# 0xMiden/miden-vm

Hardware: AMD Instinct MI355X
Metric: trace rows/sec proved (2^20-row trace, 96-bit sec) (higher is better)
Workload: dtype u64 (Goldilocks field, p = 2^64 - 2^32 + 1); 1 GPU; full proof of miden:20:51:8 (DummyMidenAir 2^20 x 51 + 8 EF aux), 96-bit production PCS params (blowup 8, FRI arity 4, 27 queries, PoW 4/12/16), Poseidon2 LMCS; trace resident in HBM, transcript on host; log_trace_rows=20, main_width=51, aux_width_ef=8, log_blowup=3, proof_bytes=137697, parallelism=1 GPU

## Files before the change

miden-vm_amd/csrc/p2_fast_constants.inc:

```
static const unsigned long long P2F_ARK_INT_SCALED[22] = {
  0x4adf842aa75d4316ULL, 0xc7ddc3945255a751ULL, 0x3a16dbc6b75abaa6ULL, 0x4160d6694e06fff1ULL,
  0xe022996682de326cULL, 0xc8e9d874293bba12ULL, 0xa2e2b15ade3b7d8fULL, 0x9b6dac180ec943cfULL,
  0xe8bb7136f94d695dULL, 0xf12458f8ebe4789bULL, 0x1dc193fff01be2b6ULL, 0xb68e807d90fed489ULL,
  0x1e4085d70c946015ULL, 0x66a5e58521b4c3c6ULL, 0x53b280ba8b2f8249ULL, 0xe4d602af8c2cf37eULL,
  0x813ee2a294c44327ULL, 0x813b943e27068773ULL, 0x9abe7bd4fb69436eULL, 0x12f583e142599766ULL,
  0x3798883e37881f6bULL, 0xed264b0c16fc039fULL,
};
static const unsigned long long P2F_INT_K[22] = {
  0x0000000000000001ULL, 0xffffbfff00004001ULL, 0xefffffff00000001ULL, 0xfffffbff00000001ULL,
  0xfffffffeff000001ULL, 0xfffffffeffffffc1ULL, 0x000ffffffff00000ULL, 0x00000003fffffffcULL,
  0x0001000000000000ULL, 0x0000000040000000ULL, 0x0000000000001000ULL, 0xfbffffff04000001ULL,
  0xfffffeff00000101ULL, 0xffbfffff00000001ULL, 0xffffffef00000001ULL, 0xfffffffefffc0001ULL,
  0xffffffff00000000ULL, 0x00003fffffffc000ULL, 0x1000000000000000ULL, 0x0000040000000000ULL,
  0x0000000001000000ULL, 0x0000000000000040ULL,
};
static const unsigned long long P2F_DESCALE = 0xfffffffec0000001ULL;
static const unsigned long long P2G_ARK[22] = {
  0x4adf842aa75d4316ULL, 0x8fbb8729a4ab4ea1ULL, 0x742db78d6eb5754cULL, 0x82c1acd29c0dffe2ULL,
  0xc04532ce05bc64d7ULL, 0x91d3b0e952777423ULL, 0x45c562b6bc76fb1dULL, 0x36db58311d92879dULL,
  0xd176e26ef29ad2b9ULL, 0xe248b1f2d7c8f135ULL, 0x3b8327ffe037c56cULL, 0x6d1d00fc21fda911ULL,
  0x3c810bae1928c02aULL, 0xcd4bcb0a4369878cULL, 0xa7650175165f0492ULL, 0xc9ac05601859e6fbULL,
  0x027dc5462988864dULL, 0x0277287d4e0d0ee5ULL, 0x357cf7aaf6d286dbULL, 0x25eb07c284b32eccULL,
  0x6f31107c6f103ed6ULL, 0xda4c96192df8073dULL,
};
static const unsigned long long P2G_K[22] = {
  0x0000000000000002ULL, 0xfffffeff00000101ULL, 0xffbfffff00000001ULL, 0xffffffef00000001ULL,
  0xfffffffefffc0001ULL, 0xffffffff00000000ULL, 0x00003fffffffc000ULL, 0x1000000000000000ULL,
  0x0000040000000000ULL, 0x0000000001000000ULL, 0x0000000000000040ULL, 0xffefffff00100001ULL,
  0xfffffffb00000005ULL, 0xfffeffff00000001ULL, 0xfffffffec0000001ULL, 0xfffffffefffff001ULL,
  0x03fffffffc000000ULL, 0x000000ffffffff00ULL, 0x0040000000000000ULL, 0x0000001000000000ULL,
  0x0000000000040000ULL, 0x0000000000000001ULL,
};
static const unsigned long long P2G_DESCALE = 0xfffffffee0000001ULL;
```

miden-vm_amd/csrc/poseidon2_fast.cuh:

```cuda
#pragma once
#include "poseidon2.cuh"

namespace p2c {
#include "p2_fast_constants.inc"
}

#ifndef P2F_ASM
#define P2F_ASM 1
#endif
#ifndef P2F_GROUP
#define P2F_GROUP 4
#endif

#if defined(__HIP_DEVICE_COMPILE__)

template <u32 K>
__device__ __forceinline__ u64 p2f_mad(u64 acc, u32 x) {
  u64 d, cy;
  asm("v_mad_u64_u32 %0, %1, %2, %3, %4" : "=v"(d), "=s"(cy) : "v"(x), "n"(K), "v"(acc));
  return d;
}
template <u32 K>
__device__ __forceinline__ u64 p2f_zmul(u32 x) {
  u64 d, cy;
  asm("v_mad_u64_u32 %0, %1, %2, %3, 0" : "=v"(d), "=s"(cy) : "v"(x), "n"(K));
  return d;
}
__device__ __forceinline__ u32 lo32(u64 x) { return (u32)x; }
__device__ __forceinline__ u32 hi32(u64 x) { return (u32)(x >> 32); }

__device__ __forceinline__ u64 p2f_mul_c(u64 a, u64 b) {
  const u32 a0 = lo32(a), a1 = hi32(a), b0 = lo32(b), b1 = hi32(b);
  const u64 p00 = (u64)a0 * b0;
  const u64 m = (u64)a0 * b1 + (p00 >> 32);
  const u64 m2 = (u64)a1 * b0 + (u32)m;
  const u64 hi = (u64)a1 * b1 + (m >> 32) + (m2 >> 32);
  const u64 lo = (m2 << 32) | (u32)p00;
  const u32 x2 = lo32(hi), x3 = hi32(hi);
  u64 t = (u64)x2 * 0xFFFFFFFFu + lo;
  t += (t < lo) ? GL_EPS : 0;
  u64 r = t - x3;
  r -= (t < x3) ? GL_EPS : 0;
  return r;
}
#define P2F_A asm volatile
#ifndef P2F_GAP_NOPS
#define P2F_GAP_NOPS 1
#endif
#define P2F_GAP()                                          \
  do {                                                     \
    if (P2F_GAP_NOPS && N == 1) P2F_A("s_nop 1");          \
    else if (P2F_GAP_NOPS && N == 2) P2F_A("s_nop 0");     \
  } while (0)
#define P2F_SCR(i, PRE, POST, ...)                                                  \
  do {                                                                              \
    switch ((i) & 7) {                                                              \
      case 0: P2F_A(PRE "s[84:85]" POST : __VA_ARGS__ : "s84", "s85"); break;        \
      case 1: P2F_A(PRE "s[86:87]" POST : __VA_ARGS__ : "s86", "s87"); break;        \
      case 2: P2F_A(PRE "s[88:89]" POST : __VA_ARGS__ : "s88", "s89"); break;        \
      case 3: P2F_A(PRE "s[90:91]" POST : __VA_ARGS__ : "s90", "s91"); break;        \
      case 4: P2F_A(PRE "s[92:93]" POST : __VA_ARGS__ : "s92", "s93"); break;        \
      case 5: P2F_A(PRE "s[94:95]" POST : __VA_ARGS__ : "s94", "s95"); break;        \
      case 6: P2F_A(PRE "s[96:97]" POST : __VA_ARGS__ : "s96", "s97"); break;        \
      default: P2F_A(PRE "s[98:99]" POST : __VA_ARGS__ : "s98", "s99"); break;       \
    }                                                                               \
  } while (0)
#define P2F_MAD0(i, D, X, Y) P2F_SCR(i, "v_mad_u64_u32 %0, ", ", %1, %2, 0", "=v"(D) : "v"(X), "v"(Y))
#define P2F_MADA(i, D, X, Y, ACC) P2F_SCR(i, "v_mad_u64_u32 %0, ", ", %1, %2, %3", "=v"(D) : "v"(X), "v"(Y), "v"(ACC))
#define P2F_CARRY_IN(i, OP, D, X, C) P2F_SCR(i, OP " %0, ", ", %1, 0, %2", "=v"(D) : "v"(X), "s"(C))
#define P2F_MAD0S(i, D, X, Y) P2F_SCR(i, "v_mad_u64_u32 %0, ", ", %1, %2, 0", "=v"(D) : "v"(X), "s"(Y))
#define P2F_MADAS(i, D, X, Y, ACC) P2F_SCR(i, "v_mad_u64_u32 %0, ", ", %1, %2, %3", "=v"(D) : "v"(X), "s"(Y), "v"(ACC))
template <int N, bool BS = false>
__device__ __forceinline__ void p2f_mulN(u64 (&r)[N], const u64 (&a)[N], const u64 (&b)[N]) {
  u64 p00[N], m[N], hi[N], t[N];
  u64 cm[N], k1[N], k2[N], k3[N], c1[N], bb[N], bw[N], c3[N];
  u32 w1[N], accl[N], acch[N], rl[N], rh[N];
#pragma unroll
  for (int i = 0; i < N; i++) {
    if constexpr (BS) P2F_MAD0S(i, p00[i], lo32(a[i]), lo32(b[i]));
    else P2F_MAD0(i, p00[i], lo32(a[i]), lo32(b[i]));
  }
#pragma unroll
  for (int i = 0; i < N; i++) {
    if constexpr (BS) P2F_MAD0S(i, m[i], lo32(a[i]), hi32(b[i]));
    else P2F_MAD0(i, m[i], lo32(a[i]), hi32(b[i]));
  }
#pragma unroll
  for (int i = 0; i < N; i++) {
    if constexpr (BS) P2F_A("v_mad_u64_u32 %0, %1, %2, %3, %4" : "=v"(m[i]), "=s"(cm[i]) : "v"(hi32(a[i])), "s"(lo32(b[i])), "0"(m[i]));
    else P2F_A("v_mad_u64_u32 %0, %1, %2, %3, %4" : "=v"(m[i]), "=s"(cm[i]) : "v"(hi32(a[i])), "v"(lo32(b[i])), "0"(m[i]));
  }
#pragma unroll
  for (int i = 0; i < N; i++) P2F_A("v_add_co_u32_e64 %0, %1, %2, %3" : "=v"(w1[i]), "=s"(k1[i]) : "v"(hi32(p00[i])), "v"(lo32(m[i])));
  P2F_GAP();
#pragma unroll
  for (int i = 0; i < N; i++) P2F_A("v_addc_co_u32_e64 %0, %1, %2, 0, %3" : "=v"(accl[i]), "=s"(k2[i]) : "v"(hi32(m[i])), "s"(k1[i]));
#pragma unroll
  for (int i = 0; i < N; i++)
    k3[i] = cm[i] | k2[i];
#pragma unroll
  for (int i = 0; i < N; i++) {
    const u32 zero = 0;
    P2F_CARRY_IN(i, "v_addc_co_u32_e64", acch[i], zero, k3[i]);
  }
#pragma unroll
  for (int i = 0; i < N; i++) {
    const u64 acc = ((u64)acch[i] << 32) | accl[i];
    if constexpr (BS) P2F_MADAS(i, hi[i], hi32(a[i]), hi32(b[i]), acc);
    else P2F_MADA(i, hi[i], hi32(a[i]), hi32(b[i]), acc);
  }
#pragma unroll
  for (int i = 0; i < N; i++) {
    const u64 lo = ((u64)w1[i] << 32) | lo32(p00[i]);
    P2F_A("v_mad_u64_u32 %0, %1, %2, -1, %3" : "=v"(t[i]), "=s"(c1[i]) : "v"(lo32(hi[i])), "v"(lo));
  }
  P2F_GAP();
#pragma unroll
  for (int i = 0; i < N; i++) P2F_A("v_subb_co_u32_e64 %0, %1, %2, %3, %4" : "=v"(rl[i]), "=s"(bb[i]) : "v"(lo32(t[i])), "v"(hi32(hi[i])), "s"(c1[i]));
#pragma unroll
  for (int i = 0; i < N; i++) P2F_CARRY_IN(i, "v_addc_co_u32_e64", rh[i], hi32(t[i]), c1[i]);
  if (P2F_GAP_NOPS && N == 1) P2F_A("s_nop 0");
#pragma unroll
  for (int i = 0; i < N; i++) P2F_A("v_subb_co_u32_e64 %0, %1, %2, 0, %3" : "=v"(rh[i]), "=s"(bw[i]) : "0"(rh[i]), "s"(bb[i]));
  P2F_GAP();
#pragma unroll
  for (int i = 0; i < N; i++) P2F_A("v_addc_co_u32_e64 %0, %1, %2, 0, %3" : "=v"(rl[i]), "=s"(c3[i]) : "0"(rl[i]), "s"(bw[i]));
#pragma unroll
  for (int i = 0; i < N; i++) k3[i] = bw[i] & ~c3[i];
#pragma unroll
  for (int i = 0; i < N; i++) {
    P2F_CARRY_IN(i, "v_subb_co_u32_e64", rh[i], rh[i], k3[i]);
    r[i] = ((u64)rh[i] << 32) | rl[i];
  }
}
#undef P2F_GAP
#undef P2F_SCR
#undef P2F_MAD0
#undef P2F_MADA
#undef P2F_MAD0S
#undef P2F_MADAS
#undef P2F_CARRY_IN
__device__ __forceinline__ u64 p2f_mul_nv(u64 a, u64 b) {
  u64 p00, m, hi, t, d0, d1, d2, d3, d4, d5, cm, k1, k2, c1, bb, bw, c3;
  u32 w1, accl, acch, rl, rh;
  const u32 zero = 0;
  asm("v_mad_u64_u32 %0, %1, %2, %3, 0" : "=v"(p00), "=s"(d0) : "v"(lo32(a)), "v"(lo32(b)));
  asm("v_mad_u64_u32 %0, %1, %2, %3, 0" : "=v"(m), "=s"(d1) : "v"(lo32(a)), "v"(hi32(b)));
  asm("v_mad_u64_u32 %0, %1, %2, %3, %4" : "=v"(m), "=s"(cm) : "v"(hi32(a)), "v"(lo32(b)), "0"(m));
  asm("v_add_co_u32_e64 %0, %1, %2, %3" : "=v"(w1), "=s"(k1) : "v"(hi32(p00)), "v"(lo32(m)));
  asm("s_nop 1\n\tv_addc_co_u32_e64 %0, %1, %2, 0, %3" : "=v"(accl), "=s"(k2) : "v"(hi32(m)), "s"(k1));
  const u64 k3 = cm | k2;
  asm("v_addc_co_u32_e64 %0, %1, %2, 0, %3" : "=v"(acch), "=s"(d2) : "v"(zero), "s"(k3));
  const u64 acc = ((u64)acch << 32) | accl;
  asm("v_mad_u64_u32 %0, %1, %2, %3, %4" : "=v"(hi), "=s"(d3) : "v"(hi32(a)), "v"(hi32(b)), "v"(acc));
  const u64 lo = ((u64)w1 << 32) | lo32(p00);
  asm("v_mad_u64_u32 %0, %1, %2, -1, %3" : "=v"(t), "=s"(c1) : "v"(lo32(hi)), "v"(lo));
  asm("s_nop 1\n\tv_subb_co_u32_e64 %0, %1, %2, %3, %4" : "=v"(rl), "=s"(bb) : "v"(lo32(t)), "v"(hi32(hi)), "s"(c1));
  asm("s_nop 1\n\tv_addc_co_u32_e64 %0, %1, %2, 0, %3" : "=v"(rh), "=s"(d4) : "v"(hi32(t)), "s"(c1));
  asm("s_nop 1\n\tv_subb_co_u32_e64 %0, %1, %2, 0, %3" : "=v"(rh), "=s"(bw) : "0"(rh), "s"(bb));
  asm("s_nop 1\n\tv_addc_co_u32_e64 %0, %1, %2, 0, %3" : "=v"(rl), "=s"(c3) : "0"(rl), "s"(bw));
  const u64 mk = bw & ~c3;
  asm("v_subb_co_u32_e64 %0, %1, %2, 0, %3" : "=v"(rh), "=s"(d5) : "0"(rh), "s"(mk));
  return ((u64)rh << 32) | rl;
}
__device__ __forceinline__ u64 p2f_mul(u64 a, u64 b) {
#if P2F_ASM
  u64 r[1];
  const u64 x[1] = {a}, y[1] = {b};
  p2f_mulN<1>(r, x, y);
  return r[0];
#else
  return p2f_mul_c(a, b);
#endif
}
__device__ __forceinline__ u64 p2f_mul_k(u64 a, u64 k) {
#if P2F_ASM
  u64 r[1];
  const u64 x[1] = {a}, y[1] = {k};
  p2f_mulN<1, true>(r, x, y);
  return r[0];
#else
  return p2f_mul_c(a, k);
#endif
}
__device__ __forceinline__ u64 p2f_sbox(u64 x) {
#if P2F_ASM
  const u64 x2 = p2f_mul(x, x);
  u64 q[2];
  const u64 qa[2] = {x2, x2}, qb[2] = {x, x2};
  p2f_mulN<2>(q, qa, qb);
  return p2f_mul(q[0], q[1]);
#else
  const u64 x2 = p2f_mul(x, x);
  const u64 x3 = p2f_mul(x2, x);
  const u64 x4 = p2f_mul(x2, x2);
  return p2f_mul(x3, x4);
#endif
}
__device__ __forceinline__ void p2f_sbox12(u64 s[12]) {
#if P2F_ASM
#pragma unroll
  for (int g = 0; g < 12; g += P2F_GROUP) {
    u64 x[P2F_GROUP], x2[P2F_GROUP], x3[P2F_GROUP];
#pragma unroll
    for (int i = 0; i < P2F_GROUP; i++) x[i] = s[g + i];
    p2f_mulN<P2F_GROUP>(x2, x, x);
    p2f_mulN<P2F_GROUP>(x3, x2, x);
    p2f_mulN<P2F_GROUP>(x, x2, x2);
    p2f_mulN<P2F_GROUP>(x2, x3, x);
#pragma unroll
    for (int i = 0; i < P2F_GROUP; i++) s[g + i] = x2[i];
  }
#else
#pragma unroll
  for (int i = 0; i < 12; i++) s[i] = p2f_sbox(s[i]);
#endif
}
__device__ __forceinline__ u64 p2f_add_canon(u64 x, u64 c) {
  u64 s = x + c;
  s += (s < c) ? GL_EPS : 0;
  return s;
}
__device__ __forceinline__ u64 p2f_fold(u64 L, u64 H) {
  const u64 m = (u64)hi32(H) * 0xFFFFFFFFu + L;
  const u32 hl = lo32(H);
  const u32 s = hi32(m) + hl;
  u64 r = ((u64)s << 32) | lo32(m);
  r += (s < hl) ? GL_EPS : 0;
  return r;
}
__device__ __forceinline__ u64 p2f_fold_signed(u64 L, u64 H) {
  const u64 BL = ((u64)1 << 30) + ((u64)1 << 62);
  const u64 BH = ((u64)1 << 30) * 0xFFFFFFFFULL - ((u64)1 << 30);
  return p2f_fold(L + BL, H + BH);
}

template <bool RC>
__device__ __forceinline__ void p2f_external(u64 s[12], const unsigned long long* rc) {
  u64 oL[12], oH[12];
#pragma unroll
  for (int i = 0; i < 12; i += 4) {
#pragma unroll
    for (int part = 0; part < 2; part++) {
      const u32 a = part ? hi32(s[i]) : lo32(s[i]), b = part ? hi32(s[i + 1]) : lo32(s[i + 1]);
      const u32 c = part ? hi32(s[i + 2]) : lo32(s[i + 2]), d = part ? hi32(s[i + 3]) : lo32(s[i + 3]);
      const u64 t01 = p2f_mad<1>(p2f_zmul<1>(a), b);
      const u64 t23 = p2f_mad<1>(p2f_zmul<1>(c), d);
      const u64 t0123 = t01 + t23;
      const u64 t01123 = p2f_mad<1>(t0123, b);
      const u64 t01233 = p2f_mad<1>(t0123, d);
      u64* o = part ? oH : oL;
      o[i + 3] = p2f_mad<2>(t01233, a);
      o[i + 1] = p2f_mad<2>(t01123, c);
      o[i] = t01123 + t01;
      o[i + 2] = t01233 + t23;
    }
  }
#pragma unroll
  for (int l = 0; l < 4; l++) {
    const u64 stL = oL[l] + oL[4 + l] + oL[8 + l], stH = oH[l] + oH[4 + l] + oH[8 + l];
#pragma unroll
    for (int i = l; i < 12; i += 4) {
      u64 L = oL[i] + stL, H = oH[i] + stH;
      if (RC) {
        L += rc[i] & 0xFFFFFFFFULL;
        H += rc[i] >> 32;
      }
      s[i] = p2f_fold(L, H);
    }
  }
}

__device__ __forceinline__ void p2f_permute(u64 s[12]) {
  p2f_external<true>(s, p2c::P2_ARK_EXT_INITIAL);
#pragma unroll 1
  for (int r = 0; r < 4; r++) {
    p2f_sbox12(s);
    if (r < 3) {
      p2f_external<true>(s, p2c::P2_ARK_EXT_INITIAL + 12 * (r + 1));
    } else {
      p2f_external<false>(s, nullptr);
    }
  }
  u64 t0 = p2f_add_canon(s[0], p2c::P2G_ARK[0]);
  u64 X1L, X1H, X2L, X2H, X11L, X11H;
  u64 AL[4], AH[4], BL[4], BH[4];
  {
    const u64 y = p2f_mul_k(p2f_sbox(t0), p2c::P2G_K[0]);
    u64 RL = p2f_zmul<1>(lo32(s[1])), RH = p2f_zmul<1>(hi32(s[1]));
#pragma unroll
    for (int i = 2; i < 12; i++) {
      RL = p2f_mad<1>(RL, lo32(s[i]));
      RH = p2f_mad<1>(RH, hi32(s[i]));
    }
    const u64 s8L = p2f_mad<1>(RL << 1, lo32(y)) << 3, s8H = p2f_mad<1>(RH << 1, hi32(y)) << 3;
    {
      const u64 rc = p2c::P2G_ARK[1];
      t0 = p2f_fold_signed((((RL << 1) - (u64)lo32(y)) << 3) + (rc & 0xFFFFFFFFULL), (((RH << 1) - (u64)hi32(y)) << 3) + (rc >> 32));
    }
    X1L = p2f_mad<16>(s8L, lo32(s[1])), X1H = p2f_mad<16>(s8H, hi32(s[1]));
    X2L = p2f_mad<32>(s8L, lo32(s[2])), X2H = p2f_mad<32>(s8H, hi32(s[2]));
    X11L = p2f_mad<2>(s8L, lo32(s[11])), X11H = p2f_mad<2>(s8H, hi32(s[11]));
#define P2G_PAIR0(q, i, j, K)                                                         \
  AL[q] = p2f_mad<1>(p2f_zmul<1>(lo32(s[i])), lo32(s[j]));                            \
  AH[q] = p2f_mad<1>(p2f_zmul<1>(hi32(s[i])), hi32(s[j]));                            \
  BL[q] = p2f_mad<K>(s8L, lo32(s[i])) - p2f_zmul<K>(lo32(s[j]));                      \
  BH[q] = p2f_mad<K>(s8H, hi32(s[i])) - p2f_zmul<K>(hi32(s[j]));
    P2G_PAIR0(0, 3, 6, 4)
    P2G_PAIR0(1, 4, 7, 24)
    P2G_PAIR0(2, 5, 8, 32)
    P2G_PAIR0(3, 9, 10, 2)
#undef P2G_PAIR0
  }
#define P2G_ROUND(r, CL, CH, PL, PH, HAS_RC)                                                             \
  {                                                                                                       \
    const u64 y = p2f_mul_k(p2f_sbox(t0), p2c::P2G_K[r]);                                                   \
    const u64 RL = ((CL[0] + CL[1] + CL[2] + CL[3]) << 1) + X1L + X2L + X11L;                             \
    const u64 RH = ((CH[0] + CH[1] + CH[2] + CH[3]) << 1) + X1H + X2H + X11H;                             \
    const u64 s8L = p2f_mad<1>(RL, lo32(y)) << 3, s8H = p2f_mad<1>(RH, hi32(y)) << 3;                     \
    {                                                                                                     \
      u64 nL = (RL - (u64)lo32(y)) << 3, nH = (RH - (u64)hi32(y)) << 3;            \
      if (HAS_RC) {                                                                                       \
        const u64 rc = p2c::P2G_ARK[(r) + 1];                                                             \
        nL += rc & 0xFFFFFFFFULL;                                                                         \
        nH += rc >> 32;                                                                                   \
      }                                                                                                   \
      t0 = p2f_fold_signed(nL, nH);                                                                       \
    }                                                                                                     \
    X1L = (X1L << 3) + s8L, X1H = (X1H << 3) + s8H;                                                       \
    X2L = (X2L << 4) + s8L, X2H = (X2H << 4) + s8H;                                                       \
    X11L += s8L, X11H += s8H;                                                                             \
    PL[0] = (PL[0] << 4) + s8L, PH[0] = (PH[0] << 4) + s8H;                                      \
    {                                                                                  \
      u64 uL, uH;  \
      asm("v_lshl_add_u64 %0, %1, 3, %1" : "=v"(uL) : "v"(PL[1]));                                        \
      asm("v_lshl_add_u64 %0, %1, 3, %1" : "=v"(uH) : "v"(PH[1]));                                        \
      PL[1] = ((uL << 2) << 4) + s8L, PH[1] = ((uH << 2) << 4) + s8H;                                     \
    }                                                                                                     \
    PL[2] = ((PL[2] << 6) << 4) + s8L, PH[2] = ((PH[2] << 6) << 4) + s8H;                       \
    PL[3] = (PL[3] << 2) + s8L, PH[3] = (PH[3] << 2) + s8H;                                      \
  }
#define P2G_REFOLD(L_, H_)                        \
  {                                               \
    const u64 v = p2f_fold_signed(L_, H_);        \
    L_ = p2f_zmul<1>(lo32(v));                    \
    H_ = p2f_zmul<1>(hi32(v));                    \
  }
#pragma unroll 1
  for (int r = 1; r < 22; r += 2) {
    P2G_ROUND(r, BL, BH, AL, AH, r < 21)
    if ((r & 3) == 3) {
      P2G_REFOLD(X1L, X1H)
      P2G_REFOLD(X2L, X2H)
      P2G_REFOLD(X11L, X11H)
#pragma unroll
      for (int q = 0; q < 4; q++) {
        P2G_REFOLD(AL[q], AH[q])
        P2G_REFOLD(BL[q], BH[q])
      }
    }
    if (r + 1 < 22) P2G_ROUND(r + 1, AL, AH, BL, BH, true)
  }
#undef P2G_ROUND
#undef P2G_REFOLD
  s[0] = t0;
  s[1] = p2f_fold_signed(X1L, X1H);
  s[2] = p2f_fold_signed(X2L, X2H);
  s[11] = p2f_fold_signed(X11L, X11H);
#define P2G_UNPAIR(q, i, j, KL, KH)                         \
  {                                                         \
    const u64 kL = KL, kH = KH;                             \
    s[i] = p2f_fold_signed(AL[q] + kL, AH[q] + kH);         \
    s[j] = p2f_fold_signed(AL[q] - kL, AH[q] - kH);         \
  }
  P2G_UNPAIR(0, 3, 6, BL[0] << 2, BH[0] << 2)
  P2G_UNPAIR(1, 4, 7, ((BL[1] << 1) + BL[1]) << 3, ((BH[1] << 1) + BH[1]) << 3)
  P2G_UNPAIR(2, 5, 8, BL[2] << 5, BH[2] << 5)
  P2G_UNPAIR(3, 9, 10, BL[3] << 1, BH[3] << 1)
#undef P2G_UNPAIR
#if P2F_ASM
#pragma unroll
  for (int g = 0; g < 12; g += 4) {
    u64 x[4], k[4];
#pragma unroll
    for (int i = 0; i < 4; i++) { x[i] = s[g + i]; k[i] = p2c::P2G_DESCALE; }
    p2f_mulN<4>(x, x, k);
#pragma unroll
    for (int i = 0; i < 4; i++) s[g + i] = x[i];
  }
#else
#pragma unroll
  for (int i = 0; i < 12; i++) s[i] = p2f_mul(s[i], p2c::P2G_DESCALE);
#endif
#pragma unroll
  for (int i = 0; i < 12; i++) s[i] = p2f_add_canon(s[i], p2c::P2_ARK_EXT_TERMINAL[i]);
#pragma unroll 1
  for (int r = 0; r < 4; r++) {
    p2f_sbox12(s);
    if (r < 3) {
      p2f_external<true>(s, p2c::P2_ARK_EXT_TERMINAL + 12 * (r + 1));
    } else {
      p2f_external<false>(s, nullptr);
    }
  }
#pragma unroll
  for (int i = 0; i < 12; i++) s[i] = gl_canon(s[i]);
}

#else
__device__ void p2f_permute(u64 s[12]);
__device__ u64 p2f_mul(u64 a, u64 b);
__device__ u64 p2f_mul_nv(u64 a, u64 b);
__device__ u64 p2f_mul_k(u64 a, u64 k);
__device__ u64 p2f_sbox(u64 x);
__device__ void p2f_sbox12(u64 s[12]);
__device__ u32 lo32(u64 x);
__device__ u32 hi32(u64 x);
#endif
```

miden-vm_amd/csrc/poseidon2_lanes.cuh:

```cuda
#pragma once
#include "poseidon2_fast.cuh"

#if defined(__HIP_DEVICE_COMPILE__)

template <int CTRL>
__device__ __forceinline__ u64 p2l_dpp(u64 v) {
  const u32 lo = (u32)__builtin_amdgcn_mov_dpp((int)lo32(v), CTRL, 0xF, 0xF, false);
  const u32 hi = (u32)__builtin_amdgcn_mov_dpp((int)hi32(v), CTRL, 0xF, 0xF, false);
  return ((u64)hi << 32) | lo;
}
#define P2L_QUAD(a, b, c, d) ((a) | ((b) << 2) | ((c) << 4) | ((d) << 6))
#define P2L_ROW_ROR(n) (0x120 + (n))
#define P2L_ROW_BCAST0 0x150

template <bool RC>
__device__ __forceinline__ u64 p2l_external(u64 s, int g, u64 c) {
  const u64 x1 = p2l_dpp<P2L_QUAD(1, 2, 3, 0)>(s), x2 = p2l_dpp<P2L_QUAD(2, 3, 0, 1)>(s), x3 = p2l_dpp<P2L_QUAD(3, 0, 1, 2)>(s);
  u64 oL = p2f_mad<2>(p2f_mad<3>(p2f_mad<1>(p2f_zmul<1>(lo32(x3)), lo32(x2)), lo32(x1)), lo32(s));
  u64 oH = p2f_mad<2>(p2f_mad<3>(p2f_mad<1>(p2f_zmul<1>(hi32(x3)), hi32(x2)), hi32(x1)), hi32(s));
  if (g >= 12) { oL = 0; oH = 0; }
  const u64 sL = oL + p2l_dpp<P2L_ROW_ROR(4)>(oL) + p2l_dpp<P2L_ROW_ROR(8)>(oL) + p2l_dpp<P2L_ROW_ROR(12)>(oL);
  const u64 sH = oH + p2l_dpp<P2L_ROW_ROR(4)>(oH) + p2l_dpp<P2L_ROW_ROR(8)>(oH) + p2l_dpp<P2L_ROW_ROR(12)>(oH);
  u64 L = oL + sL, H = oH + sH;
  if (RC) {
    L += c & 0xFFFFFFFFULL;
    H += c >> 32;
  }
  return p2f_fold(L, H);
}

__device__ __forceinline__ u64 p2l_permute(u64 s) {
  const int lane = threadIdx.x & 63, g = lane & 15;
  const int gi = g < 12 ? g : 0;
  u64 rci[4], rct[4];
#pragma unroll
  for (int k = 0; k < 4; k++) {
    rci[k] = p2c::P2_ARK_EXT_INITIAL[12 * k + gi];
    rct[k] = p2c::P2_ARK_EXT_TERMINAL[12 * k + gi];
  }
  s = p2l_external<true>(s, g, rci[0]);
#pragma unroll
  for (int r = 0; r < 4; r++) {
    s = p2f_sbox(s);
    s = r < 3 ? p2l_external<true>(s, g, rci[r + 1]) : p2l_external<false>(s, g, 0);
  }
  const u64 mag_lo = 0x1804201804100810ULL, mag_hi = 0x0000000001020220ULL;
  const u32 neg_bits = 0x5C1;
  const u64 mag = ((g < 8 ? mag_lo : mag_hi) >> (8 * (g & 7))) & 0xff;
  const u64 sgn = ((neg_bits >> g) & 1) ? ~(u64)0 : 0;
  u64 t0 = p2f_add_canon(s, p2c::P2F_ARK_INT_SCALED[0]);
  u64 L = (g >= 1 && g < 12) ? (u64)lo32(s) : 0, H = (g >= 1 && g < 12) ? (u64)hi32(s) : 0;
  u64 nL = 0, nH = 0;
  u64 k_cur = p2c::P2F_INT_K[0], a_cur = p2c::P2F_ARK_INT_SCALED[1];
#pragma unroll 1
  for (int r = 0; r < 22; r++) {
    const u64 k_nxt = p2c::P2F_INT_K[r < 21 ? r + 1 : 21], a_nxt = p2c::P2F_ARK_INT_SCALED[r < 20 ? r + 2 : 21];
    u64 sL = L, sH = H;
    sL += p2l_dpp<P2L_ROW_ROR(8)>(sL); sH += p2l_dpp<P2L_ROW_ROR(8)>(sH);
    sL += p2l_dpp<P2L_ROW_ROR(4)>(sL); sH += p2l_dpp<P2L_ROW_ROR(4)>(sH);
    sL += p2l_dpp<P2L_QUAD(2, 3, 0, 1)>(sL); sH += p2l_dpp<P2L_QUAD(2, 3, 0, 1)>(sH);
    sL += p2l_dpp<P2L_QUAD(1, 0, 3, 2)>(sL); sH += p2l_dpp<P2L_QUAD(1, 0, 3, 2)>(sH);
    const u64 mL = L * mag, mH = H * mag;
    const u64 cL = (mL ^ sgn) - sgn, cH = (mH ^ sgn) - sgn;
    const u64 y = p2l_dpp<P2L_ROW_BCAST0>(p2f_mul(p2f_sbox(t0), k_cur));
    const u64 yl = lo32(y), yh = hi32(y);
    sL += yl;
    sH += yh;
    L = (sL << 3) + cL;
    H = (sH << 3) + cH;
    nL = (sL << 3) - (yl << 4);
    nH = (sH << 3) - (yh << 4);
    if (g == 0 || g >= 12) { L = 0; H = 0; }
    if (r < 21) t0 = p2f_fold_signed(nL + (a_cur & 0xFFFFFFFFULL), nH + (a_cur >> 32));
    k_cur = k_nxt;
    a_cur = a_nxt;
    if ((r & 3) == 3) {
      const u64 v = p2f_fold_signed(L, H);
      L = lo32(v);
      H = hi32(v);
      if (g == 0 || g >= 12) { L = 0; H = 0; }
    }
  }
  if (g == 0) {
    L = nL;
    H = nH;
  }
  s = p2f_add_canon(p2f_mul(p2f_fold_signed(L, H), p2c::P2F_DESCALE), rct[0]);
#pragma unroll
  for (int r = 0; r < 4; r++) {
    s = p2f_sbox(s);
    s = r < 3 ? p2l_external<true>(s, g, rct[r + 1]) : p2l_external<false>(s, g, 0);
  }
  return gl_canon(s);
}

#else
__device__ u64 p2l_permute(u64 s);
#endif
```

miden-vm_amd/csrc/poseidon2_quad.cuh:

```cuda
#pragma once
#include "poseidon2_lanes.cuh"

#if defined(__HIP_DEVICE_COMPILE__)

template <bool RC>
__device__ __forceinline__ void p2q_external(u64 (&s)[3], const u64 (&c)[3]) {
  u64 oL[3], oH[3];
#pragma unroll
  for (int k = 0; k < 3; k++) {
    const u64 x1 = p2l_dpp<P2L_QUAD(1, 2, 3, 0)>(s[k]), x2 = p2l_dpp<P2L_QUAD(2, 3, 0, 1)>(s[k]), x3 = p2l_dpp<P2L_QUAD(3, 0, 1, 2)>(s[k]);
    oL[k] = p2f_mad<2>(p2f_mad<3>(p2f_mad<1>(p2f_zmul<1>(lo32(x3)), lo32(x2)), lo32(x1)), lo32(s[k]));
    oH[k] = p2f_mad<2>(p2f_mad<3>(p2f_mad<1>(p2f_zmul<1>(hi32(x3)), hi32(x2)), hi32(x1)), hi32(s[k]));
  }
  const u64 sL = oL[0] + oL[1] + oL[2], sH = oH[0] + oH[1] + oH[2];
#pragma unroll
  for (int k = 0; k < 3; k++) {
    u64 L = oL[k] + sL, H = oH[k] + sH;
    if (RC) {
      L += c[k] & 0xFFFFFFFFULL;
      H += c[k] >> 32;
    }
    s[k] = p2f_fold(L, H);
  }
}

__device__ __forceinline__ void p2q_sbox3(u64 (&s)[3]) {
  u64 x2[3], x3[3], x4[3];
  p2f_mulN<3>(x2, s, s);
  p2f_mulN<3>(x3, x2, s);
  p2f_mulN<3>(x4, x2, x2);
  p2f_mulN<3>(s, x3, x4);
}

__device__ __forceinline__ void p2q_permute(u64 (&s)[3]) {
  const int j = threadIdx.x & 3;
  u64 rci[4][3], rct[4][3];
#pragma unroll
  for (int r = 0; r < 4; r++)
#pragma unroll
    for (int k = 0; k < 3; k++) {
      rci[r][k] = p2c::P2_ARK_EXT_INITIAL[12 * r + 4 * k + j];
      rct[r][k] = p2c::P2_ARK_EXT_TERMINAL[12 * r + 4 * k + j];
    }
  p2q_external<true>(s, rci[0]);
#pragma unroll
  for (int r = 0; r < 4; r++) {
    p2q_sbox3(s);
    if (r < 3) p2q_external<true>(s, rci[r + 1]);
    else p2q_external<false>(s, rci[0]);
  }
  const u64 mag_lo = 0x1804201804100810ULL, mag_hi = 0x0000000001020220ULL;
  const u32 neg_bits = 0x5C1;
  u64 mag[3], sgn[3], L[3], H[3];
#pragma unroll
  for (int k = 0; k < 3; k++) {
    const int e = 4 * k + j;
    mag[k] = ((e < 8 ? mag_lo : mag_hi) >> (8 * (e & 7))) & 0xff;
    sgn[k] = ((neg_bits >> e) & 1) ? ~(u64)0 : 0;
    L[k] = lo32(s[k]);
    H[k] = hi32(s[k]);
  }
  u64 t0 = p2f_add_canon(s[0], p2c::P2F_ARK_INT_SCALED[0]);
  if (j == 0) { L[0] = 0; H[0] = 0; }
  u64 k_cur = p2c::P2F_INT_K[0], a_cur = p2c::P2F_ARK_INT_SCALED[1];
#pragma unroll 1
  for (int r = 0; r < 22; r++) {
    const u64 k_nxt = p2c::P2F_INT_K[r < 21 ? r + 1 : 21], a_nxt = p2c::P2F_ARK_INT_SCALED[r < 20 ? r + 2 : 21];
    const u64 y = p2l_dpp<P2L_QUAD(0, 0, 0, 0)>(p2f_mul(p2f_sbox(t0), k_cur));
    if (j == 0) {
      L[0] = lo32(y);
      H[0] = hi32(y);
    }
    u64 sL = L[0] + L[1] + L[2], sH = H[0] + H[1] + H[2];
    sL += p2l_dpp<P2L_QUAD(1, 0, 3, 2)>(sL); sH += p2l_dpp<P2L_QUAD(1, 0, 3, 2)>(sH);
    sL += p2l_dpp<P2L_QUAD(2, 3, 0, 1)>(sL); sH += p2l_dpp<P2L_QUAD(2, 3, 0, 1)>(sH);
#pragma unroll
    for (int k = 0; k < 3; k++) {
      const u64 mL = L[k] * mag[k], mH = H[k] * mag[k];
      L[k] = (sL << 3) + ((mL ^ sgn[k]) - sgn[k]);
      H[k] = (sH << 3) + ((mH ^ sgn[k]) - sgn[k]);
    }
    u64 nL = L[0], nH = H[0];
    if (r < 21) {
      nL += a_cur & 0xFFFFFFFFULL;
      nH += a_cur >> 32;
    }
    t0 = p2f_fold_signed(nL, nH);
    k_cur = k_nxt;
    a_cur = a_nxt;
    if ((r & 3) == 3) {
#pragma unroll
      for (int k = 0; k < 3; k++) {
        const u64 v = p2f_fold_signed(L[k], H[k]);
        L[k] = lo32(v);
        H[k] = hi32(v);
      }
    }
  }
#pragma unroll
  for (int k = 0; k < 3; k++) s[k] = p2f_add_canon(p2f_mul(p2f_fold_signed(L[k], H[k]), p2c::P2F_DESCALE), rct[0][k]);
#pragma unroll
  for (int r = 0; r < 4; r++) {
    p2q_sbox3(s);
    if (r < 3) p2q_external<true>(s, rct[r + 1]);
    else p2q_external<false>(s, rct[0]);
  }
#pragma unroll
  for (int k = 0; k < 3; k++) s[k] = gl_canon(s[k]);
}

#else
__device__ void p2q_permute(u64 (&s)[3]);
#endif
```

Baseline: 22.73 million trace rows/s.

## Replace internal-round constant multiplies with power-of-two shift accumulation and full unroll

The internal-round constants of Poseidon2 are powers of two modulo Goldilocks, so the field multiply of the S-box output by K is replaced by a compile-time shift that splits the value into three 32-bit words. Those words are added or subtracted into the lazy L/H accumulators with signs chosen at compile time, using 2^96 = -1. The 22-round internal loops in the scalar, lanes and quad permutations are fully unrolled through constexpr lambdas so exponents and round constants become immediates. This removes a 64-bit modular multiply per round on the serial critical path, at the cost of larger code and more register pressure from the unrolling.

```diff
diff --git a/miden-vm_amd/csrc/p2_fast_constants.inc b/miden-vm_amd/csrc/p2_fast_constants.inc
--- a/miden-vm_amd/csrc/p2_fast_constants.inc
+++ b/miden-vm_amd/csrc/p2_fast_constants.inc
@@ -32,3 +32,7 @@
   0x0000000000040000ULL, 0x0000000000000001ULL,
 };
 static const unsigned long long P2G_DESCALE = 0xfffffffee0000001ULL;
+static constexpr int P2F_INT_K_LOG2[22] = {0, 174, 156, 138, 120, 102, 84, 66, 48, 30, 12, 186, 168, 150, 132, 114, 96, 78, 60, 42, 24, 6};
+static constexpr int P2F_DESCALE_LOG2 = 126;
+static constexpr int P2G_K_LOG2[22] = {1, 168, 150, 132, 114, 96, 78, 60, 42, 24, 6, 180, 162, 144, 126, 108, 90, 72, 54, 36, 18, 0};
+static constexpr int P2G_DESCALE_LOG2 = 125;
diff --git a/miden-vm_amd/csrc/poseidon2_fast.cuh b/miden-vm_amd/csrc/poseidon2_fast.cuh
--- a/miden-vm_amd/csrc/poseidon2_fast.cuh
+++ b/miden-vm_amd/csrc/poseidon2_fast.cuh
@@ -235,6 +235,53 @@
   return p2f_fold(L + BL, H + BH);
 }
 
+__host__ __device__ constexpr int p2f_shl_sign(int E, int part, int w) {
+  constexpr int tab[3][2][3] = {{{1, 0, -1}, {0, 1, 1}}, {{0, -1, -1}, {1, 1, 0}}, {{-1, -1, 0}, {1, 0, -1}}};
+  const int e = E % 96, sg = tab[e / 32][part][w] * (E >= 96 ? -1 : 1);
+  return (w == 2 && e % 32 == 0) ? 0 : sg;
+}
+template <int E>
+__device__ __forceinline__ void p2f_shl_words(u64 y, u32 (&u)[3]) {
+  static_assert(E >= 0 && E < 192, "exponent out of range");
+  constexpr int b = E % 96 % 32;
+  const u64 z = y << b;
+  u[0] = lo32(z);
+  u[1] = hi32(z);
+  if constexpr (b > 0) u[2] = hi32(y) >> (32 - b);
+  else u[2] = 0;
+}
+template <int SG>
+__device__ __forceinline__ u64 p2f_acc_word(u64 acc, u32 u) {
+  if constexpr (SG > 0) return p2f_mad<1>(acc, u);
+  else if constexpr (SG < 0) return acc - (u64)u;
+  else return acc;
+}
+template <int E, int PART, int SG>
+__device__ __forceinline__ u64 p2f_acc_shl(u64 acc, const u32 (&u)[3]) {
+  acc = p2f_acc_word<SG * p2f_shl_sign(E, PART, 0)>(acc, u[0]);
+  acc = p2f_acc_word<SG * p2f_shl_sign(E, PART, 1)>(acc, u[1]);
+  return p2f_acc_word<SG * p2f_shl_sign(E, PART, 2)>(acc, u[2]);
+}
+#define P2F_IC(F, r) F(std::integral_constant<int, r>{})
+#define P2F_ROUNDS22(F)                                                                                               \
+  do {                                                                                                                \
+    P2F_IC(F, 0); P2F_IC(F, 1); P2F_IC(F, 2); P2F_IC(F, 3); P2F_IC(F, 4); P2F_IC(F, 5); P2F_IC(F, 6); P2F_IC(F, 7);          \
+    P2F_IC(F, 8); P2F_IC(F, 9); P2F_IC(F, 10); P2F_IC(F, 11); P2F_IC(F, 12); P2F_IC(F, 13); P2F_IC(F, 14); P2F_IC(F, 15);    \
+    P2F_IC(F, 16); P2F_IC(F, 17); P2F_IC(F, 18); P2F_IC(F, 19); P2F_IC(F, 20); P2F_IC(F, 21);                             \
+  } while (0)
+template <int E, int PART>
+__device__ __forceinline__ void p2f_pm_shl(u64 R, const u32 (&u)[3], u64& s8, u64& n) {
+  constexpr int plus = (p2f_shl_sign(E, PART, 0) > 0) + (p2f_shl_sign(E, PART, 1) > 0) + (p2f_shl_sign(E, PART, 2) > 0);
+  constexpr int minus = (p2f_shl_sign(E, PART, 0) < 0) + (p2f_shl_sign(E, PART, 1) < 0) + (p2f_shl_sign(E, PART, 2) < 0);
+  if constexpr (plus >= minus) {
+    s8 = p2f_acc_shl<E, PART, 1>(R, u) << 3;
+    n = (R << 4) - s8;
+  } else {
+    n = p2f_acc_shl<E, PART, -1>(R, u) << 3;
+    s8 = (R << 4) - n;
+  }
+}
+
 template <bool RC>
 __device__ __forceinline__ void p2f_external(u64 s[12], const unsigned long long* rc) {
   u64 oL[12], oH[12];
@@ -286,17 +333,20 @@
   u64 X1L, X1H, X2L, X2H, X11L, X11H;
   u64 AL[4], AH[4], BL[4], BH[4];
   {
-    const u64 y = p2f_mul_k(p2f_sbox(t0), p2c::P2G_K[0]);
+    u32 y[3];
+    p2f_shl_words<p2c::P2G_K_LOG2[0]>(p2f_sbox(t0), y);
     u64 RL = p2f_zmul<1>(lo32(s[1])), RH = p2f_zmul<1>(hi32(s[1]));
 #pragma unroll
     for (int i = 2; i < 12; i++) {
       RL = p2f_mad<1>(RL, lo32(s[i]));
       RH = p2f_mad<1>(RH, hi32(s[i]));
     }
-    const u64 s8L = p2f_mad<1>(RL << 1, lo32(y)) << 3, s8H = p2f_mad<1>(RH << 1, hi32(y)) << 3;
+    u64 s8L, s8H, nL, nH;
+    p2f_pm_shl<p2c::P2G_K_LOG2[0], 0>(RL << 1, y, s8L, nL);
+    p2f_pm_shl<p2c::P2G_K_LOG2[0], 1>(RH << 1, y, s8H, nH);
     {
       const u64 rc = p2c::P2G_ARK[1];
-      t0 = p2f_fold_signed((((RL << 1) - (u64)lo32(y)) << 3) + (rc & 0xFFFFFFFFULL), (((RH << 1) - (u64)hi32(y)) << 3) + (rc >> 32));
+      t0 = p2f_fold_signed(nL + (rc & 0xFFFFFFFFULL), nH + (rc >> 32));
     }
     X1L = p2f_mad<16>(s8L, lo32(s[1])), X1H = p2f_mad<16>(s8H, hi32(s[1]));
     X2L = p2f_mad<32>(s8L, lo32(s[2])), X2H = p2f_mad<32>(s8H, hi32(s[2]));
@@ -314,12 +364,14 @@
   }
 #define P2G_ROUND(r, CL, CH, PL, PH, HAS_RC)                                                             \
   {                                                                                                       \
-    const u64 y = p2f_mul_k(p2f_sbox(t0), p2c::P2G_K[r]);                                                   \
+    u32 y[3];                            \
+    p2f_shl_words<p2c::P2G_K_LOG2[r]>(p2f_sbox(t0), y);                                                   \
     const u64 RL = ((CL[0] + CL[1] + CL[2] + CL[3]) << 1) + X1L + X2L + X11L;                             \
     const u64 RH = ((CH[0] + CH[1] + CH[2] + CH[3]) << 1) + X1H + X2H + X11H;                             \
-    const u64 s8L = p2f_mad<1>(RL, lo32(y)) << 3, s8H = p2f_mad<1>(RH, hi32(y)) << 3;                     \
+    u64 s8L, s8H, nL, nH;                                 \
+    p2f_pm_shl<p2c::P2G_K_LOG2[r], 0>(RL, y, s8L, nL);                                                    \
+    p2f_pm_shl<p2c::P2G_K_LOG2[r], 1>(RH, y, s8H, nH);                                                    \
     {                                                                                                     \
-      u64 nL = (RL - (u64)lo32(y)) << 3, nH = (RH - (u64)hi32(y)) << 3;            \
       if (HAS_RC) {                                                                                       \
         const u64 rc = p2c::P2G_ARK[(r) + 1];                                                             \
         nL += rc & 0xFFFFFFFFULL;                                                                         \
@@ -346,10 +398,10 @@
     L_ = p2f_zmul<1>(lo32(v));                    \
     H_ = p2f_zmul<1>(hi32(v));                    \
   }
-#pragma unroll 1
-  for (int r = 1; r < 22; r += 2) {
+  const auto round_pair = [&](auto rr) {
+    constexpr int r = decltype(rr)::value;
     P2G_ROUND(r, BL, BH, AL, AH, r < 21)
-    if ((r & 3) == 3) {
+    if constexpr ((r & 3) == 3) {
       P2G_REFOLD(X1L, X1H)
       P2G_REFOLD(X2L, X2H)
       P2G_REFOLD(X11L, X11H)
@@ -359,8 +411,19 @@
         P2G_REFOLD(BL[q], BH[q])
       }
     }
-    if (r + 1 < 22) P2G_ROUND(r + 1, AL, AH, BL, BH, true)
-  }
+    if constexpr (r + 1 < 22) P2G_ROUND(r + 1, AL, AH, BL, BH, true)
+  };
+  round_pair(std::integral_constant<int, 1>{});
+  round_pair(std::integral_constant<int, 3>{});
+  round_pair(std::integral_constant<int, 5>{});
+  round_pair(std::integral_constant<int, 7>{});
+  round_pair(std::integral_constant<int, 9>{});
+  round_pair(std::integral_constant<int, 11>{});
+  round_pair(std::integral_constant<int, 13>{});
+  round_pair(std::integral_constant<int, 15>{});
+  round_pair(std::integral_constant<int, 17>{});
+  round_pair(std::integral_constant<int, 19>{});
+  round_pair(std::integral_constant<int, 21>{});
 #undef P2G_ROUND
 #undef P2G_REFOLD
   s[0] = t0;
diff --git a/miden-vm_amd/csrc/poseidon2_lanes.cuh b/miden-vm_amd/csrc/poseidon2_lanes.cuh
--- a/miden-vm_amd/csrc/poseidon2_lanes.cuh
+++ b/miden-vm_amd/csrc/poseidon2_lanes.cuh
@@ -51,10 +51,8 @@
   u64 t0 = p2f_add_canon(s, p2c::P2F_ARK_INT_SCALED[0]);
   u64 L = (g >= 1 && g < 12) ? (u64)lo32(s) : 0, H = (g >= 1 && g < 12) ? (u64)hi32(s) : 0;
   u64 nL = 0, nH = 0;
-  u64 k_cur = p2c::P2F_INT_K[0], a_cur = p2c::P2F_ARK_INT_SCALED[1];
-#pragma unroll 1
-  for (int r = 0; r < 22; r++) {
-    const u64 k_nxt = p2c::P2F_INT_K[r < 21 ? r + 1 : 21], a_nxt = p2c::P2F_ARK_INT_SCALED[r < 20 ? r + 2 : 21];
+  const auto round = [&](auto rr) {
+    constexpr int r = decltype(rr)::value, E = p2c::P2F_INT_K_LOG2[r];
     u64 sL = L, sH = H;
     sL += p2l_dpp<P2L_ROW_ROR(8)>(sL); sH += p2l_dpp<P2L_ROW_ROR(8)>(sH);
     sL += p2l_dpp<P2L_ROW_ROR(4)>(sL); sH += p2l_dpp<P2L_ROW_ROR(4)>(sH);
@@ -62,25 +60,26 @@
     sL += p2l_dpp<P2L_QUAD(1, 0, 3, 2)>(sL); sH += p2l_dpp<P2L_QUAD(1, 0, 3, 2)>(sH);
     const u64 mL = L * mag, mH = H * mag;
     const u64 cL = (mL ^ sgn) - sgn, cH = (mH ^ sgn) - sgn;
-    const u64 y = p2l_dpp<P2L_ROW_BCAST0>(p2f_mul(p2f_sbox(t0), k_cur));
-    const u64 yl = lo32(y), yh = hi32(y);
-    sL += yl;
-    sH += yh;
-    L = (sL << 3) + cL;
-    H = (sH << 3) + cH;
-    nL = (sL << 3) - (yl << 4);
-    nH = (sH << 3) - (yh << 4);
+    u32 y[3];
+    p2f_shl_words<E>(p2l_dpp<P2L_ROW_BCAST0>(p2f_sbox(t0)), y);
+    u64 s8L, s8H;
+    p2f_pm_shl<E, 0>(sL, y, s8L, nL);
+    p2f_pm_shl<E, 1>(sH, y, s8H, nH);
+    L = s8L + cL;
+    H = s8H + cH;
     if (g == 0 || g >= 12) { L = 0; H = 0; }
-    if (r < 21) t0 = p2f_fold_signed(nL + (a_cur & 0xFFFFFFFFULL), nH + (a_cur >> 32));
-    k_cur = k_nxt;
-    a_cur = a_nxt;
-    if ((r & 3) == 3) {
+    if constexpr (r < 21) {
+      const u64 a = p2c::P2F_ARK_INT_SCALED[r + 1];
+      t0 = p2f_fold_signed(nL + (a & 0xFFFFFFFFULL), nH + (a >> 32));
+    }
+    if constexpr ((r & 3) == 3) {
       const u64 v = p2f_fold_signed(L, H);
       L = lo32(v);
       H = hi32(v);
       if (g == 0 || g >= 12) { L = 0; H = 0; }
     }
-  }
+  };
+  P2F_ROUNDS22(round);
   if (g == 0) {
     L = nL;
     H = nH;
diff --git a/miden-vm_amd/csrc/poseidon2_quad.cuh b/miden-vm_amd/csrc/poseidon2_quad.cuh
--- a/miden-vm_amd/csrc/poseidon2_quad.cuh
+++ b/miden-vm_amd/csrc/poseidon2_quad.cuh
@@ -62,14 +62,13 @@
   }
   u64 t0 = p2f_add_canon(s[0], p2c::P2F_ARK_INT_SCALED[0]);
   if (j == 0) { L[0] = 0; H[0] = 0; }
-  u64 k_cur = p2c::P2F_INT_K[0], a_cur = p2c::P2F_ARK_INT_SCALED[1];
-#pragma unroll 1
-  for (int r = 0; r < 22; r++) {
-    const u64 k_nxt = p2c::P2F_INT_K[r < 21 ? r + 1 : 21], a_nxt = p2c::P2F_ARK_INT_SCALED[r < 20 ? r + 2 : 21];
-    const u64 y = p2l_dpp<P2L_QUAD(0, 0, 0, 0)>(p2f_mul(p2f_sbox(t0), k_cur));
+  const auto round = [&](auto rr) {
+    constexpr int r = decltype(rr)::value, E = p2c::P2F_INT_K_LOG2[r];
+    u32 y[3];
+    p2f_shl_words<E>(p2l_dpp<P2L_QUAD(0, 0, 0, 0)>(p2f_sbox(t0)), y);
     if (j == 0) {
-      L[0] = lo32(y);
-      H[0] = hi32(y);
+      L[0] = p2f_acc_shl<E, 0, 1>(0, y);
+      H[0] = p2f_acc_shl<E, 1, 1>(0, y);
     }
     u64 sL = L[0] + L[1] + L[2], sH = H[0] + H[1] + H[2];
     sL += p2l_dpp<P2L_QUAD(1, 0, 3, 2)>(sL); sH += p2l_dpp<P2L_QUAD(1, 0, 3, 2)>(sH);
@@ -81,14 +80,13 @@
       H[k] = (sH << 3) + ((mH ^ sgn[k]) - sgn[k]);
     }
     u64 nL = L[0], nH = H[0];
-    if (r < 21) {
-      nL += a_cur & 0xFFFFFFFFULL;
-      nH += a_cur >> 32;
+    if constexpr (r < 21) {
+      const u64 a = p2c::P2F_ARK_INT_SCALED[r + 1];
+      nL += a & 0xFFFFFFFFULL;
+      nH += a >> 32;
     }
     t0 = p2f_fold_signed(nL, nH);
-    k_cur = k_nxt;
-    a_cur = a_nxt;
-    if ((r & 3) == 3) {
+    if constexpr ((r & 3) == 3) {
 #pragma unroll
       for (int k = 0; k < 3; k++) {
         const u64 v = p2f_fold_signed(L[k], H[k]);
@@ -96,7 +94,8 @@
         H[k] = hi32(v);
       }
     }
-  }
+  };
+  P2F_ROUNDS22(round);
 #pragma unroll
   for (int k = 0; k < 3; k++) s[k] = p2f_add_canon(p2f_mul(p2f_fold_signed(L[k], H[k]), p2c::P2F_DESCALE), rct[0][k]);
 #pragma unroll
```

Result: faster. 23.41 million trace rows/s, median of 6 (+3.0%).
